# Edward-Sun/DIFUSCO

Hardware: NVIDIA H100
Metric: TSP-500 graphs/sec, 50-step categorical denoise (higher is better)
Workload: dtype f32 (3-term bf16 split on wgmma, fp32 accumulate)

## Files before the change

difusco_b200/csrc/edge_layer_tc.cuh:

```cuda
#pragma once
#include <cuda.h>
#include <cuda_bf16.h>
#include <cuda_runtime.h>

#include <stdlib.h>

#include <string>

#include "common.cuh"
#include "edge_layer_fp32.cuh"

namespace dfb {

constexpr int WG_ROWS = 64;
constexpr int TC_KCH = 64;
constexpr int TC_B_BYTES = 256 * 128;
constexpr int TC_A_CHUNK = WG_ROWS * 128;
constexpr int TC_A_BYTES = 8 * TC_A_CHUNK;
constexpr int CONV_BATCH = 16;

constexpr int W_LO_ROWS = H;
constexpr int W_MAT_ROWS = 2 * W_LO_ROWS;
constexpr int W_LAYER_ROWS = 6 * W_MAT_ROWS;
__host__ __device__ constexpr int w_row_C(int l) { return l * W_LAYER_ROWS; }
__host__ __device__ constexpr int w_row_O(int l) { return w_row_C(l) + W_MAT_ROWS; }
__host__ __device__ constexpr int w_row_UVAB(int l) { return w_row_C(l) + 2 * W_MAT_ROWS; }
__host__ __device__ constexpr int w_row_embed(int L, int which) { return L * W_LAYER_ROWS + which * W_MAT_ROWS; }
__host__ __device__ constexpr int w_arena_rows(int L) { return w_row_embed(L, 2); }

template <int NWG>
struct TcCfg {
  static_assert(NWG == 1 || NWG == 2, "one or two consumer warpgroups");
  static constexpr int TILE = NWG * WG_ROWS;
  static constexpr int THREADS = (NWG + 1) * 128;
  static constexpr int NSTAGE = (NWG == 1) ? 3 : 2;
  static constexpr int OFF_B = NWG * TC_A_BYTES;
  static constexpr int OFF_PRM = OFF_B + NSTAGE * TC_B_BYTES;
  static constexpr int OFF_ROW = OFF_PRM + 6 * H * 4;
  static constexpr int OFF_SRC = OFF_ROW + TILE * 4;
  static constexpr int OFF_BAR = OFF_SRC + TILE * 8;
  static constexpr int SMEM_BYTES = OFF_BAR + 2 * NSTAGE * 8;
  static constexpr int SMEM_ALLOC = SMEM_BYTES + 1024;
  static constexpr int OFF_TAU = SMEM_BYTES;
  static constexpr int SMEM_ALLOC_TROWS = SMEM_ALLOC + TILE * 8;
  static_assert(SMEM_ALLOC_TROWS <= 232448, "shared memory budget (227 KB per block)");
};

struct TcParams {
  float* e;
  const float* uvab;
  float* partials;
  GraphDev g;
  LayerParams lp;
  const float* tvec;
  const float* xt_lut;
  const float* lut;
  const float* zero_row;
  float* debug_acc;
  const float* lin_in;
  float* lin_out;
  const float* lin_bias;
  int lin_rows;
  int lin_nb;
  int lin_w_row;
  int* error_flag;
  unsigned long long* phase_cycles;
  int write_e, e_zero, agg_mode;
  int w_row_base;
  int n_tiles;
  TimeRows trows;
};

__device__ __forceinline__ uint32_t smem_u32(const void* p) { return (uint32_t)__cvta_generic_to_shared(p); }

__device__ __forceinline__ void mbar_init(uint64_t* bar, uint32_t count) {
  asm volatile("mbarrier.init.shared::cta.b64 [%0], %1;" ::"r"(smem_u32(bar)), "r"(count) : "memory");
}
__device__ __forceinline__ void mbar_arrive(uint64_t* bar) {
  asm volatile("mbarrier.arrive.shared::cta.b64 _, [%0];" ::"r"(smem_u32(bar)) : "memory");
}
__device__ __forceinline__ void mbar_arrive_expect_tx(uint64_t* bar, uint32_t bytes) {
  asm volatile("mbarrier.arrive.expect_tx.shared::cta.b64 _, [%0], %1;" ::"r"(smem_u32(bar)), "r"(bytes) : "memory");
}
__device__ __forceinline__ void mbar_wait(uint64_t* bar, uint32_t parity, int* error_flag, int code) {
  const uint32_t addr = smem_u32(bar);
  uint32_t ok = 0;
#pragma unroll 1
  for (uint32_t spin = 0;; ++spin) {
    asm volatile(
        "{\n .reg .pred p;\n mbarrier.try_wait.parity.shared::cta.b64 p, [%1], %2, %3;\n selp.u32 %0, 1, 0, p;\n}"
        : "=r"(ok)
        : "r"(addr), "r"(parity), "r"(20000u)
        : "memory");
    if (ok) return;
    if (spin > 400000u) {
      if (error_flag) {
        error_flag[1] = (int)blockIdx.x;
        error_flag[2] = (int)parity;
        error_flag[3] = (int)threadIdx.x;
        atomicExch(error_flag, code);
      }
      __threadfence_system();
      __trap();
    }
  }
}
__device__ __forceinline__ void tma_load_2d(uint32_t dst, const CUtensorMap* map, uint64_t* bar, int c0, int c1) {
  asm volatile(
      "cp.async.bulk.tensor.2d.shared::cluster.global.mbarrier::complete_tx::bytes [%0], [%1, {%3, %4}], [%2];"
      ::"r"(dst), "l"(reinterpret_cast<uint64_t>(map)), "r"(smem_u32(bar)), "r"(c0), "r"(c1)
      : "memory");
}
__device__ __forceinline__ void fence_proxy_async() { asm volatile("fence.proxy.async.shared::cta;" ::: "memory"); }
__device__ __forceinline__ void cp_async16(void* dst, const void* src) {
  asm volatile("cp.async.cg.shared.global [%0], [%1], 16;" ::"r"(smem_u32(dst)), "l"(src) : "memory");
}
__device__ __forceinline__ void cp_async_commit() { asm volatile("cp.async.commit_group;" ::: "memory"); }
__device__ __forceinline__ void cp_async_wait_all() { asm volatile("cp.async.wait_group 0;" ::: "memory"); }

__device__ __forceinline__ uint64_t wgmma_desc_sw128(uint32_t smem_addr) {
  return (uint64_t)((smem_addr >> 4) & 0x3fffu) | (1ull << 16) | (64ull << 32) | (1ull << 62);
}
__device__ __forceinline__ void wgmma_fence() { asm volatile("wgmma.fence.sync.aligned;" ::: "memory"); }
__device__ __forceinline__ void wgmma_commit() { asm volatile("wgmma.commit_group.sync.aligned;" ::: "memory"); }
template <int N>
__device__ __forceinline__ void wgmma_wait() { asm volatile("wgmma.wait_group.sync.aligned %0;" ::"n"(N) : "memory"); }
__device__ __forceinline__ void acc_fence(float (&d)[128]) {
#pragma unroll
  for (int i = 0; i < 128; ++i) asm volatile("" : "+f"(d[i])::"memory");
}
__device__ __forceinline__ void wgmma_bf16(float (&d)[128], uint64_t da, uint64_t db, uint32_t scale_d) {
  asm volatile(
      "{\n .reg .pred p;\n setp.ne.b32 p, %130, 0;\n"
      "wgmma.mma_async.sync.aligned.m64n256k16.f32.bf16.bf16 "
      "{%0, %1, %2, %3, %4, %5, %6, %7, %8, %9, %10, %11, %12, %13, %14, %15, "
      "%16, %17, %18, %19, %20, %21, %22, %23, %24, %25, %26, %27, %28, %29, %30, %31, "
      "%32, %33, %34, %35, %36, %37, %38, %39, %40, %41, %42, %43, %44, %45, %46, %47, "
      "%48, %49, %50, %51, %52, %53, %54, %55, %56, %57, %58, %59, %60, %61, %62, %63, "
      "%64, %65, %66, %67, %68, %69, %70, %71, %72, %73, %74, %75, %76, %77, %78, %79, "
      "%80, %81, %82, %83, %84, %85, %86, %87, %88, %89, %90, %91, %92, %93, %94, %95, "
      "%96, %97, %98, %99, %100, %101, %102, %103, %104, %105, %106, %107, %108, %109, %110, %111, "
      "%112, %113, %114, %115, %116, %117, %118, %119, %120, %121, %122, %123, %124, %125, %126, %127}, "
      "%128, %129, p, 1, 1, 0, 0;\n}"
      : "+f"(d[0]), "+f"(d[1]), "+f"(d[2]), "+f"(d[3]), "+f"(d[4]), "+f"(d[5]), "+f"(d[6]), "+f"(d[7]),
        "+f"(d[8]), "+f"(d[9]), "+f"(d[10]), "+f"(d[11]), "+f"(d[12]), "+f"(d[13]), "+f"(d[14]), "+f"(d[15]),
        "+f"(d[16]), "+f"(d[17]), "+f"(d[18]), "+f"(d[19]), "+f"(d[20]), "+f"(d[21]), "+f"(d[22]), "+f"(d[23]),
        "+f"(d[24]), "+f"(d[25]), "+f"(d[26]), "+f"(d[27]), "+f"(d[28]), "+f"(d[29]), "+f"(d[30]), "+f"(d[31]),
        "+f"(d[32]), "+f"(d[33]), "+f"(d[34]), "+f"(d[35]), "+f"(d[36]), "+f"(d[37]), "+f"(d[38]), "+f"(d[39]),
        "+f"(d[40]), "+f"(d[41]), "+f"(d[42]), "+f"(d[43]), "+f"(d[44]), "+f"(d[45]), "+f"(d[46]), "+f"(d[47]),
        "+f"(d[48]), "+f"(d[49]), "+f"(d[50]), "+f"(d[51]), "+f"(d[52]), "+f"(d[53]), "+f"(d[54]), "+f"(d[55]),
        "+f"(d[56]), "+f"(d[57]), "+f"(d[58]), "+f"(d[59]), "+f"(d[60]), "+f"(d[61]), "+f"(d[62]), "+f"(d[63]),
        "+f"(d[64]), "+f"(d[65]), "+f"(d[66]), "+f"(d[67]), "+f"(d[68]), "+f"(d[69]), "+f"(d[70]), "+f"(d[71]),
        "+f"(d[72]), "+f"(d[73]), "+f"(d[74]), "+f"(d[75]), "+f"(d[76]), "+f"(d[77]), "+f"(d[78]), "+f"(d[79]),
        "+f"(d[80]), "+f"(d[81]), "+f"(d[82]), "+f"(d[83]), "+f"(d[84]), "+f"(d[85]), "+f"(d[86]), "+f"(d[87]),
        "+f"(d[88]), "+f"(d[89]), "+f"(d[90]), "+f"(d[91]), "+f"(d[92]), "+f"(d[93]), "+f"(d[94]), "+f"(d[95]),
        "+f"(d[96]), "+f"(d[97]), "+f"(d[98]), "+f"(d[99]), "+f"(d[100]), "+f"(d[101]), "+f"(d[102]), "+f"(d[103]),
        "+f"(d[104]), "+f"(d[105]), "+f"(d[106]), "+f"(d[107]), "+f"(d[108]), "+f"(d[109]), "+f"(d[110]), "+f"(d[111]),
        "+f"(d[112]), "+f"(d[113]), "+f"(d[114]), "+f"(d[115]), "+f"(d[116]), "+f"(d[117]), "+f"(d[118]), "+f"(d[119]),
        "+f"(d[120]), "+f"(d[121]), "+f"(d[122]), "+f"(d[123]), "+f"(d[124]), "+f"(d[125]), "+f"(d[126]), "+f"(d[127])
      : "l"(da), "l"(db), "r"(scale_d));
}

__device__ __forceinline__ float sigmoid_mufu(float x) {
  float t, r;
  asm("ex2.approx.ftz.f32 %0, %1;" : "=f"(t) : "f"(-1.4426950408889634f * x));
  asm("rcp.approx.ftz.f32 %0, %1;" : "=f"(r) : "f"(1.0f + t));
  return r;
}
__device__ __forceinline__ void split4(float4 x, uint2& hi, uint2& lo) {
  __nv_bfloat162 h01 = __floats2bfloat162_rn(x.x, x.y), h23 = __floats2bfloat162_rn(x.z, x.w);
  float2 f01 = __bfloat1622float2(h01), f23 = __bfloat1622float2(h23);
  __nv_bfloat162 l01 = __floats2bfloat162_rn(x.x - f01.x, x.y - f01.y);
  __nv_bfloat162 l23 = __floats2bfloat162_rn(x.z - f23.x, x.w - f23.y);
  hi.x = *reinterpret_cast<uint32_t*>(&h01);
  hi.y = *reinterpret_cast<uint32_t*>(&h23);
  lo.x = *reinterpret_cast<uint32_t*>(&l01);
  lo.y = *reinterpret_cast<uint32_t*>(&l23);
}
__device__ __forceinline__ void split2(float a, float b, uint32_t& hi, uint32_t& lo) {
  __nv_bfloat162 h = __floats2bfloat162_rn(a, b);
  const float2 f = __bfloat1622float2(h);
  __nv_bfloat162 l = __floats2bfloat162_rn(a - f.x, b - f.y);
  hi = *reinterpret_cast<uint32_t*>(&h);
  lo = *reinterpret_cast<uint32_t*>(&l);
}
__device__ __forceinline__ uint32_t sw128_off(int r, int j) {
  return (uint32_t)((r >> 3) * 1024 + (r & 7) * 128 + ((j ^ (r & 7)) << 4));
}
__device__ __forceinline__ int msg_col(int j, int r) { return 64 * (j >> 3) + ((8 * (j & 7)) ^ (8 * (r & 7))); }
__device__ __forceinline__ float quad_sum(float v) {
  v += __shfl_xor_sync(0xffffffffu, v, 1);
  return v + __shfl_xor_sync(0xffffffffu, v, 2);
}
__device__ __forceinline__ void swap_row_halves(float (&d)[128]) {
#pragma unroll
  for (int j = 0; j < 32; ++j) {
    const float x0 = d[4 * j], x1 = d[4 * j + 1];
    d[4 * j] = d[4 * j + 2];
    d[4 * j + 1] = d[4 * j + 3];
    d[4 * j + 2] = x0;
    d[4 * j + 3] = x1;
  }
}

enum {
  PH_TILES = 0,
  PH_TOTAL,
  PH_CONVERT,
  PH_G1_WAIT,
  PH_G1_MMA,
  PH_E1,
  PH_REDUCE,
  PH_LN,
  PH_G2_WAIT,
  PH_G2_MMA,
  PH_E4,
  PH_COUNT
};

template <int NWG, bool LIN, bool TIMED = false, bool TROWS = false>
__device__ __forceinline__ void edge_layer_wg_body(const CUtensorMap& wmap, const TcParams& P) {
  using Cfg = TcCfg<NWG>;
  constexpr int NSTAGE = Cfg::NSTAGE;
  extern __shared__ unsigned char smem_raw[];
  unsigned char* smem = smem_raw + ((1024u - (smem_u32(smem_raw) & 1023u)) & 1023u);
  float* prm = reinterpret_cast<float*>(smem + Cfg::OFF_PRM);
  int* s_row = reinterpret_cast<int*>(smem + Cfg::OFF_ROW);
  const float** s_src = reinterpret_cast<const float**>(smem + Cfg::OFF_SRC);
  const float** s_tau = reinterpret_cast<const float**>(smem + Cfg::OFF_TAU);
  uint64_t* full = reinterpret_cast<uint64_t*>(smem + Cfg::OFF_BAR);
  uint64_t* empty = full + NSTAGE;

  const int warp = threadIdx.x >> 5, lane = threadIdx.x & 31;
  constexpr bool lin = LIN;
  const int loads_per_tile = (P.write_e ? 16 : 8) * NWG;

  if (threadIdx.x == 0) {
    for (int s = 0; s < NSTAGE; ++s) {
      mbar_init(&full[s], 1);
      mbar_init(&empty[s], 4);
    }
    asm volatile("fence.mbarrier_init.release.cluster;" ::: "memory");
    fence_proxy_async();
  }
  for (int i = threadIdx.x; i < H; i += Cfg::THREADS) {
    prm[i] = P.lp.ln_e_g[i];
    prm[H + i] = P.lp.ln_e_b[i];
    prm[2 * H + i] = P.tvec ? P.tvec[i] : 0.0f;
    prm[3 * H + i] = P.lp.ln_o_g[i];
    prm[4 * H + i] = P.lp.ln_o_b[i];
    prm[5 * H + i] = P.lp.b_O[i];
  }
  __syncthreads();
  const uint32_t smem_base = smem_u32(smem);

  if (warp >= 4 * NWG) {
    if constexpr (NWG == 2) asm volatile("setmaxnreg.dec.sync.aligned.u32 40;" ::: "memory");
    if (warp == 4 * NWG && lane == 0) {
      uint32_t u = 0;
      for (int tile = blockIdx.x; tile < P.n_tiles; tile += gridDim.x) {
        for (int i = 0; i < loads_per_tile; ++i, ++u) {
          const int s = u % NSTAGE;
          mbar_wait(&empty[s], ((u / NSTAGE) & 1) ^ 1, P.error_flag, 1);
          mbar_arrive_expect_tx(&full[s], TC_B_BYTES);
          const int row = (lin ? P.lin_w_row + (P.lin_nb == 4 ? (tile & 3) : 0) * W_MAT_ROWS
                               : P.w_row_base + (i >= 8 * NWG ? w_row_O(0) - w_row_C(0) : 0)) +
                          (i & 1) * W_LO_ROWS;
          tma_load_2d(smem_base + Cfg::OFF_B + s * TC_B_BYTES, &wmap, &full[s], ((i >> 1) & 3) * TC_KCH, row);
        }
      }
    }
    return;
  }

  if constexpr (NWG == 2) asm volatile("setmaxnreg.inc.sync.aligned.u32 232;" ::: "memory");
  const int wg = warp >> 2, wi = warp & 3, tid = threadIdx.x & 127;
  const int t4 = lane & 3;
  const int lr0 = wi * 16 + (lane >> 2);
  unsigned char* a_reg = smem + wg * TC_A_BYTES;
  const uint32_t a_base = smem_base + wg * TC_A_BYTES;
  float* msg = reinterpret_cast<float*>(a_reg);
  int* w_row = s_row + wg * WG_ROWS;
  const float** w_src = s_src + wg * WG_ROWS;
  const float** w_tau = s_tau + wg * WG_ROWS;
  auto wg_bar = [&] { asm volatile("bar.sync %0, 128;" ::"r"(1 + wg) : "memory"); };
  const int n_rows = lin ? P.lin_rows : P.g.E;
  uint32_t u = 0;
  float acc[128];

  auto turn_wait = [&] {
    if constexpr (NWG == 2) asm volatile("bar.sync %0, 256;" ::"r"(3 + wg) : "memory");
  };
  auto turn_pass = [&] {
    if constexpr (NWG == 2) asm volatile("bar.arrive %0, 256;" ::"r"(4 - wg) : "memory");
  };
  if (wg == 1) turn_pass();

  uint32_t t_mark = 0, t_start = 0;
  if constexpr (TIMED) t_start = t_mark = (uint32_t)clock();
  auto record = [&](int slot, uint32_t v) {
    if constexpr (TIMED) {
      if (tid == 0) atomicAdd(P.phase_cycles + slot, (unsigned long long)v);
    }
  };
  auto mark = [&](int slot) {
    if constexpr (TIMED) {
      const uint32_t now = (uint32_t)clock();
      record(slot, now - t_mark);
      t_mark = now;
    }
  };

  auto gemm = [&](int wait_slot, int mma_slot) {
    uint32_t waited = 0;
    turn_wait();
    if constexpr (TIMED) t_mark = (uint32_t)clock();
    acc_fence(acc);
    wgmma_fence();
    int s_prev = 0;
#pragma unroll
    for (int i = 0; i < 8; ++i, ++u) {
      const int s = u % NSTAGE;
      uint32_t w0 = 0;
      if constexpr (TIMED) w0 = (uint32_t)clock();
      mbar_wait(&full[s], (u / NSTAGE) & 1, P.error_flag, 2);
      if constexpr (TIMED) waited += (uint32_t)clock() - w0;
      const uint32_t b = smem_base + Cfg::OFF_B + s * TC_B_BYTES;
      const uint32_t ahi = a_base + (i >> 1) * 2 * TC_A_CHUNK, alo = ahi + TC_A_CHUNK;
#pragma unroll
      for (int ks = 0; ks < 4; ++ks) {
        const uint64_t db = wgmma_desc_sw128(b + ks * 32);
        wgmma_bf16(acc, wgmma_desc_sw128(ahi + ks * 32), db, (i | ks) ? 1u : 0u);
        if ((i & 1) == 0) wgmma_bf16(acc, wgmma_desc_sw128(alo + ks * 32), db, 1u);
      }
      wgmma_commit();
      if (i > 0) {
        wgmma_wait<1>();
        __syncwarp();
        if (lane == 0) mbar_arrive(&empty[s_prev]);
      }
      s_prev = s;
    }
    wgmma_wait<0>();
    acc_fence(acc);
    __syncwarp();
    if (lane == 0) mbar_arrive(&empty[s_prev]);
    turn_pass();
    if constexpr (TIMED) {
      const uint32_t now = (uint32_t)clock();
      record(wait_slot, waited);
      record(mma_slot, now - t_mark - waited);
      t_mark = now;
    }
  };

  auto stage_rows = [&](auto row_src) {
#pragma unroll 1
    for (int i = 0; i < 16; ++i) {
      const int r = wi * 16 + i;
      const float* src = row_src(i) + 4 * lane;
      float* dst = msg + r * H + ((4 * lane) ^ (8 * (r & 7)));
      cp_async16(dst, src);
      cp_async16(dst + 128, src + 128);
    }
    cp_async_commit();
  };

  for (int tile = blockIdx.x; tile < P.n_tiles; tile += gridDim.x) {
    record(PH_TILES, 1);
    const int row_tile = (lin && P.lin_nb == 4) ? (tile >> 2) : tile;
    const int s_base = row_tile * Cfg::TILE + wg * WG_ROWS;
    if (tid < WG_ROWS) {
      const int s = s_base + tid;
      const float* src = P.zero_row;
      int rw = -1;
      if (s < n_rows && lin) {
        src = P.lin_in + (size_t)s * H;
      } else if (s < n_rows) {
        rw = P.g.row[s];
        if (P.e_zero) src = P.zero_row;
        else if (P.xt_lut) src = P.lut + ((P.xt_lut[P.g.perm ? P.g.perm[s] : s] != 0.0f) ? H : 0);
        else src = P.e + (size_t)s * H;
      }
      w_row[tid] = rw;
      w_src[tid] = src;
      if constexpr (TROWS) w_tau[tid] = s < n_rows ? time_row(P.tvec, P.trows, P.g.perm ? P.g.perm[s] : s) : P.zero_row;
    }
    wg_bar();

#pragma unroll 1
    for (int it0 = 0; it0 < 32; it0 += CONV_BATCH) {
      float4 x[CONV_BATCH];
#pragma unroll
      for (int q = 0; q < CONV_BATCH; ++q) {
        const int item = (it0 + q) * 128 + tid;
        x[q] = __ldcg(reinterpret_cast<const float4*>(w_src[item >> 6]) + (item & 63));
      }
#pragma unroll
      for (int q = 0; q < CONV_BATCH; ++q) {
        const int item = (it0 + q) * 128 + tid;
        const int rr = item >> 6, k4 = item & 63;
        uint2 hi, lo;
        split4(x[q], hi, lo);
        const uint32_t off = (k4 >> 4) * 2 * TC_A_CHUNK + sw128_off(rr, (k4 & 15) >> 1) + (k4 & 1) * 8;
        *reinterpret_cast<uint2*>(a_reg + off) = hi;
        *reinterpret_cast<uint2*>(a_reg + off + TC_A_CHUNK) = lo;
      }
    }
    fence_proxy_async();
    wg_bar();
    mark(PH_CONVERT);
    gemm(PH_G1_WAIT, PH_G1_MMA);

    const int sa = s_base + lr0, sb = sa + 8;
    const bool va = sa < n_rows, vb = sb < n_rows;
    if (lin || P.debug_acc) {
      const int nb = (lin && P.lin_nb == 4) ? (tile & 3) : 0;
      const int ostride = lin ? P.lin_nb * H : H;
      float* out = lin ? P.lin_out + nb * H : P.debug_acc;
#pragma unroll
      for (int h = 0; h < 2; ++h) {
        const int s = h ? sb : sa;
        if (!(h ? vb : va)) continue;
#pragma unroll
        for (int j = 0; j < 32; ++j) {
          const int c = 8 * j + 2 * t4;
          float2 o = make_float2(acc[4 * j + 2 * h], acc[4 * j + 2 * h + 1]);
          if (lin) {
            const float2 bb = __ldg(reinterpret_cast<const float2*>(P.lin_bias + nb * H + c));
            o.x += bb.x;
            o.y += bb.y;
          }
          __stcg(reinterpret_cast<float2*>(out + (size_t)s * ostride + c), o);
        }
      }
      continue;
    }

    const int s_lane = s_base + wi * 16 + (lane & 15);
    const int col_lane = s_lane < n_rows ? P.g.col[s_lane] : 0;
    stage_rows([&](int i) { return P.uvab + (size_t)__shfl_sync(0xffffffffu, col_lane, i) * 4 * H + H; });
#pragma unroll 1
    for (int h = 0; h < 2; ++h) {
      const bool v = h ? vb : va;
      const float* ap = P.uvab + (size_t)__shfl_sync(0xffffffffu, col_lane, (lane >> 2) + 8 * h) * 4 * H + 2 * H;
      const float* bp = P.uvab + (size_t)(v ? P.g.row[h ? sb : sa] : 0) * 4 * H + 3 * H;
#pragma unroll
      for (int j = 0; j < 32; ++j) {
        const int c = 8 * j + 2 * t4;
        const float2 ah = __ldg(reinterpret_cast<const float2*>(ap + c));
        const float2 bh = __ldg(reinterpret_cast<const float2*>(bp + c));
        acc[4 * j] = (acc[4 * j] + ah.x) + bh.x;
        acc[4 * j + 1] = (acc[4 * j + 1] + ah.y) + bh.y;
      }
      if (h == 0) {
        cp_async_wait_all();
        __syncwarp();
      }
      float* m = msg + (lr0 + 8 * h) * H + 2 * t4;
#pragma unroll
      for (int j = 0; j < 32; ++j) {
        float2* mp = reinterpret_cast<float2*>(m + msg_col(j, lr0));
        const float2 vh = *mp;
        *mp = make_float2(sigmoid_mufu(acc[4 * j]) * vh.x, sigmoid_mufu(acc[4 * j + 1]) * vh.y);
      }
      swap_row_halves(acc);
    }
    wg_bar();
    mark(PH_E1);
    const bool amax = P.agg_mode == AGG_MAX;
    const float run0 = amax ? -INFINITY : 0.0f;
#pragma unroll 1
    for (int g2 = 0; g2 < WG_ROWS / GROUP; ++g2) {
      const int grp = (s_base >> 5) + g2;
      if (grp >= P.g.n_groups) break;
      const int first_node = P.g.grp_first[grp];
      const size_t pair_base = (size_t)P.g.grp_pair[grp];
      const int node = w_row[g2 * GROUP + lane];
      const int nxt = __shfl_down_sync(0xffffffffu, node, 1);
      const uint32_t ends = __ballot_sync(0xffffffffu, node >= 0 && (lane == GROUP - 1 || nxt != node));
#pragma unroll 1
      for (int cc = 0; cc < 2; ++cc) {
        const int c = tid + 128 * cc;
        float run = run0;
#pragma unroll 8
        for (int r = 0; r < GROUP; ++r) {
          const int lr = g2 * GROUP + r;
          const float m = msg[lr * H + (c ^ (8 * (lr & 7)))];
          run = amax ? fmaxf(run, m) : run + m;
          if ((ends >> r) & 1u) {
            P.partials[(pair_base + (size_t)(w_row[lr] - first_node)) * H + c] = run;
            run = run0;
          }
        }
      }
    }
    wg_bar();
    mark(PH_REDUCE);
    if (!P.write_e) continue;

#pragma unroll 1
    for (int h = 0; h < 2; ++h) {
      float sum = 0.f;
#pragma unroll
      for (int j = 0; j < 32; ++j) sum += acc[4 * j] + acc[4 * j + 1];
      float mean = quad_sum(sum) * (1.0f / H);
      float q = 0.f;
#pragma unroll
      for (int j = 0; j < 32; ++j) {
        const float d0 = acc[4 * j] - mean, d1 = acc[4 * j + 1] - mean;
        q = fmaf(d0, d0, fmaf(d1, d1, q));
      }
      float rstd = rsqrtf(quad_sum(q) * (1.0f / H) + LN_EPS);
      sum = 0.f;
      const float* tau = nullptr;
      if constexpr (TROWS) tau = w_tau[lr0 + 8 * h];
#pragma unroll
      for (int j = 0; j < 32; ++j) {
        const int c = 8 * j + 2 * t4;
        const float2 g = *reinterpret_cast<const float2*>(prm + c);
        const float2 b = *reinterpret_cast<const float2*>(prm + H + c);
        float2 t;
        if constexpr (TROWS) t = __ldg(reinterpret_cast<const float2*>(tau + c));
        else t = *reinterpret_cast<const float2*>(prm + 2 * H + c);
        const float y0 = fmaxf(fmaf((acc[4 * j] - mean) * rstd, g.x, b.x), 0.0f) + t.x;
        const float y1 = fmaxf(fmaf((acc[4 * j + 1] - mean) * rstd, g.y, b.y), 0.0f) + t.y;
        acc[4 * j] = y0;
        acc[4 * j + 1] = y1;
        sum += y0 + y1;
      }
      mean = quad_sum(sum) * (1.0f / H);
      q = 0.f;
#pragma unroll
      for (int j = 0; j < 32; ++j) {
        const float d0 = acc[4 * j] - mean, d1 = acc[4 * j + 1] - mean;
        q = fmaf(d0, d0, fmaf(d1, d1, q));
      }
      rstd = rsqrtf(quad_sum(q) * (1.0f / H) + LN_EPS);
      const int r = lr0 + 8 * h;
#pragma unroll
      for (int j = 0; j < 32; ++j) {
        const int c = 8 * j + 2 * t4;
        const float2 g = *reinterpret_cast<const float2*>(prm + 3 * H + c);
        const float2 b = *reinterpret_cast<const float2*>(prm + 4 * H + c);
        const float z0 = fmaf((acc[4 * j] - mean) * rstd, g.x, b.x);
        const float z1 = fmaf((acc[4 * j + 1] - mean) * rstd, g.y, b.y);
        uint32_t hi, lo;
        split2(z0 * sigmoid_mufu(z0), z1 * sigmoid_mufu(z1), hi, lo);
        const uint32_t off = (j >> 3) * 2 * TC_A_CHUNK + sw128_off(r, j & 7) + 4 * t4;
        *reinterpret_cast<uint32_t*>(a_reg + off) = hi;
        *reinterpret_cast<uint32_t*>(a_reg + off + TC_A_CHUNK) = lo;
      }
      swap_row_halves(acc);
    }
    const float* e_src = w_src[wi * 16 + (lane & 15)];
    fence_proxy_async();
    wg_bar();
    mark(PH_LN);
    gemm(PH_G2_WAIT, PH_G2_MMA);

    stage_rows([&](int i) {
      return reinterpret_cast<const float*>(__shfl_sync(0xffffffffu, reinterpret_cast<unsigned long long>(e_src), i));
    });
    cp_async_wait_all();
    __syncwarp();
#pragma unroll
    for (int h = 0; h < 2; ++h) {
      if (!(h ? vb : va)) continue;
      const int r = lr0 + 8 * h;
      const float* er = msg + r * H + 2 * t4;
      float* dst = P.e + (size_t)(h ? sb : sa) * H;
#pragma unroll
      for (int j = 0; j < 32; ++j) {
        const int c = 8 * j + 2 * t4;
        const float2 ein = *reinterpret_cast<const float2*>(er + msg_col(j, r));
        const float2 bo = *reinterpret_cast<const float2*>(prm + 5 * H + c);
        __stcg(reinterpret_cast<float2*>(dst + c),
               make_float2((ein.x + acc[4 * j + 2 * h]) + bo.x, (ein.y + acc[4 * j + 2 * h + 1]) + bo.y));
      }
    }
    mark(PH_E4);
  }
  if constexpr (TIMED) record(PH_TOTAL, (uint32_t)clock() - t_start);
}

__global__ void __launch_bounds__(TcCfg<2>::THREADS, 1)
k_edge_layer_wg2(const __grid_constant__ CUtensorMap wmap, const TcParams P) {
  edge_layer_wg_body<2, false>(wmap, P);
}
__global__ void __launch_bounds__(TcCfg<2>::THREADS, 1)
k_edge_layer_wg2_timed(const __grid_constant__ CUtensorMap wmap, const TcParams P) {
  edge_layer_wg_body<2, false, true>(wmap, P);
}
__global__ void __launch_bounds__(TcCfg<1>::THREADS, 1)
k_edge_layer_wg1(const __grid_constant__ CUtensorMap wmap, const TcParams P) {
  edge_layer_wg_body<1, false>(wmap, P);
}
__global__ void __launch_bounds__(TcCfg<2>::THREADS, 1)
k_edge_layer_wg2_trows(const __grid_constant__ CUtensorMap wmap, const TcParams P) {
  edge_layer_wg_body<2, false, false, true>(wmap, P);
}
__global__ void __launch_bounds__(TcCfg<1>::THREADS, 1)
k_edge_layer_wg1_trows(const __grid_constant__ CUtensorMap wmap, const TcParams P) {
  edge_layer_wg_body<1, false, false, true>(wmap, P);
}
__global__ void __launch_bounds__(TcCfg<2>::THREADS, 1)
k_linear_wg2(const __grid_constant__ CUtensorMap wmap, const TcParams P) {
  edge_layer_wg_body<2, true>(wmap, P);
}

struct TcState {
  std::string err;
  int num_sms = 0;
  CUtensorMap wmap;
  bool bound = false;
  float* zero_row = nullptr;
  int* error_flag = nullptr;
  int* error_host = nullptr;
  unsigned long long* phase_cycles = nullptr;

  TcState() = default;
  TcState(const TcState&) = delete;
  TcState& operator=(const TcState&) = delete;
  ~TcState() {
    if (zero_row) cudaFree(zero_row);
    if (error_host) cudaFreeHost(error_host);
    if (phase_cycles) cudaFree(phase_cycles);
  }
};

typedef CUresult (*PFN_encodeTiled)(CUtensorMap*, CUtensorMapDataType, cuuint32_t, void*, const cuuint64_t*,
                                    const cuuint64_t*, const cuuint32_t*, const cuuint32_t*, CUtensorMapInterleave,
                                    CUtensorMapSwizzle, CUtensorMapL2promotion, CUtensorMapFloatOOBfill);

inline int tc_init(TcState* st, int num_sms) {
  st->num_sms = num_sms;
  cudaError_t e = cudaFuncSetAttribute(k_edge_layer_wg2, cudaFuncAttributeMaxDynamicSharedMemorySize, TcCfg<2>::SMEM_ALLOC);
  if (e == cudaSuccess)
    e = cudaFuncSetAttribute(k_edge_layer_wg2_timed, cudaFuncAttributeMaxDynamicSharedMemorySize, TcCfg<2>::SMEM_ALLOC);
  if (e == cudaSuccess)
    e = cudaFuncSetAttribute(k_edge_layer_wg1, cudaFuncAttributeMaxDynamicSharedMemorySize, TcCfg<1>::SMEM_ALLOC);
  if (e == cudaSuccess)
    e = cudaFuncSetAttribute(k_edge_layer_wg2_trows, cudaFuncAttributeMaxDynamicSharedMemorySize, TcCfg<2>::SMEM_ALLOC_TROWS);
  if (e == cudaSuccess)
    e = cudaFuncSetAttribute(k_edge_layer_wg1_trows, cudaFuncAttributeMaxDynamicSharedMemorySize, TcCfg<1>::SMEM_ALLOC_TROWS);
  if (e == cudaSuccess)
    e = cudaFuncSetAttribute(k_linear_wg2, cudaFuncAttributeMaxDynamicSharedMemorySize, TcCfg<2>::SMEM_ALLOC);
  if (e != cudaSuccess) {
    st->err = std::string("cudaFuncSetAttribute: ") + cudaGetErrorString(e);
    return -2;
  }
  if ((e = cudaMalloc(&st->zero_row, H * sizeof(float))) != cudaSuccess ||
      (e = cudaMemset(st->zero_row, 0, H * sizeof(float))) != cudaSuccess ||
      (e = cudaMalloc(&st->phase_cycles, 32 * sizeof(unsigned long long))) != cudaSuccess ||
      (e = cudaMemset(st->phase_cycles, 0, 32 * sizeof(unsigned long long))) != cudaSuccess ||
      (e = cudaHostAlloc(&st->error_host, 4 * sizeof(int), cudaHostAllocMapped)) != cudaSuccess ||
      (e = cudaHostGetDevicePointer((void**)&st->error_flag, st->error_host, 0)) != cudaSuccess) {
    st->err = std::string("tc_init alloc: ") + cudaGetErrorString(e);
    return -2;
  }
  return 0;
}

inline int tc_bind_weights(TcState* st, const uint16_t* arena, int L) {
  void* fn = nullptr;
  cudaDriverEntryPointQueryResult qres;
  cudaError_t e = cudaGetDriverEntryPoint("cuTensorMapEncodeTiled", &fn, cudaEnableDefault, &qres);
  if (e != cudaSuccess || !fn || qres != cudaDriverEntryPointSuccess) {
    st->err = "cuTensorMapEncodeTiled entry point not available";
    cudaGetLastError();
    return -2;
  }
  cuuint64_t gdim[2] = {(cuuint64_t)H, (cuuint64_t)w_arena_rows(L)};
  cuuint64_t gstride[1] = {(cuuint64_t)H * sizeof(uint16_t)};
  cuuint32_t box[2] = {(cuuint32_t)TC_KCH, 256u};
  cuuint32_t estr[2] = {1u, 1u};
  CUresult r = ((PFN_encodeTiled)fn)(&st->wmap, CU_TENSOR_MAP_DATA_TYPE_BFLOAT16, 2, (void*)arena, gdim,
                                     gstride, box, estr, CU_TENSOR_MAP_INTERLEAVE_NONE, CU_TENSOR_MAP_SWIZZLE_128B,
                                     CU_TENSOR_MAP_L2_PROMOTION_L2_256B, CU_TENSOR_MAP_FLOAT_OOB_FILL_NONE);
  if (r != CUDA_SUCCESS) {
    st->err = "cuTensorMapEncodeTiled failed with CUresult " + std::to_string((int)r);
    return -2;
  }
  st->bound = true;
  return 0;
}

template <int NWG>
inline int tc_launch(TcState* st, void (*kernel)(CUtensorMap, TcParams), TcParams& P, int rows, int nb,
                     cudaStream_t stream, int smem = TcCfg<NWG>::SMEM_ALLOC) {
  if (!st->bound) {
    st->err = "weights not bound";
    return -1;
  }
  P.zero_row = st->zero_row; P.error_flag = st->error_flag; P.phase_cycles = st->phase_cycles;
  P.n_tiles = nb * ((rows + TcCfg<NWG>::TILE - 1) / TcCfg<NWG>::TILE);
  const int grid = P.n_tiles < st->num_sms ? P.n_tiles : st->num_sms;
  kernel<<<grid, TcCfg<NWG>::THREADS, smem, stream>>>(st->wmap, P);
  const cudaError_t err = cudaGetLastError();
  if (err == cudaSuccess) return 0;
  st->err = std::string("launch: ") + cudaGetErrorString(err);
  return -2;
}

inline int tc_launch_edge_layer(TcState* st, int l, float* e, const float* uvab, float* partials, const GraphDev& g,
                                const LayerParams& lp, const float* tvec, const TimeRows& trows, int write_e,
                                int e_zero, const float* xt_lut, const float* lut, int agg_mode, int nwg, bool timed,
                                float* debug_acc, cudaStream_t stream) {
  TcParams P{};
  P.e = e; P.uvab = uvab; P.partials = partials; P.g = g; P.lp = lp; P.tvec = tvec;
  P.xt_lut = xt_lut; P.lut = lut; P.debug_acc = debug_acc;
  P.write_e = debug_acc ? 0 : write_e;
  P.e_zero = e_zero; P.agg_mode = agg_mode;
  P.w_row_base = w_row_C(l);
  if (trows.index && tvec && !debug_acc) {
    P.trows = trows;
    if (nwg == 1) return tc_launch<1>(st, k_edge_layer_wg1_trows, P, g.E, 1, stream, TcCfg<1>::SMEM_ALLOC_TROWS);
    return tc_launch<2>(st, k_edge_layer_wg2_trows, P, g.E, 1, stream, TcCfg<2>::SMEM_ALLOC_TROWS);
  }
  if (nwg == 1) return tc_launch<1>(st, k_edge_layer_wg1, P, g.E, 1, stream);
  return tc_launch<2>(st, timed && !debug_acc ? k_edge_layer_wg2_timed : k_edge_layer_wg2, P, g.E, 1, stream);
}

inline int tc_launch_linear(TcState* st, const float* in, float* out, const float* bias, int rows, int nb, int w_row,
                            cudaStream_t stream) {
  TcParams P{};
  P.lin_in = in; P.lin_out = out; P.lin_bias = bias; P.lin_rows = rows; P.lin_nb = nb; P.lin_w_row = w_row;
  P.lp.ln_e_g = P.lp.ln_e_b = P.lp.ln_o_g = P.lp.ln_o_b = P.lp.b_O = st->zero_row;
  return tc_launch<2>(st, k_linear_wg2, P, rows, nb, stream);
}

}
```

Before: 22.44.

## Split weight TMA chunks into 32-wide K slices with a four-stage ring

```diff
diff --git a/difusco_b200/csrc/edge_layer_tc.cuh b/difusco_b200/csrc/edge_layer_tc.cuh
--- a/difusco_b200/csrc/edge_layer_tc.cuh
+++ b/difusco_b200/csrc/edge_layer_tc.cuh
@@ -13,8 +13,10 @@
 namespace dfb {
 
 constexpr int WG_ROWS = 64;
-constexpr int TC_KCH = 64;
-constexpr int TC_B_BYTES = 256 * 128;
+constexpr int TC_KBLK = 64;
+constexpr int TC_KCH = 32;
+constexpr int TC_B_BYTES = 256 * TC_KCH * 2;
+static_assert(TC_KCH * 2 == 64, "weight chunk rows are one 64-byte swizzle row (tensor map, wgmma_desc_sw64)");
 constexpr int TC_A_CHUNK = WG_ROWS * 128;
 constexpr int TC_A_BYTES = 8 * TC_A_CHUNK;
 constexpr int CONV_BATCH = 16;
@@ -33,7 +35,7 @@
   static_assert(NWG == 1 || NWG == 2, "one or two consumer warpgroups");
   static constexpr int TILE = NWG * WG_ROWS;
   static constexpr int THREADS = (NWG + 1) * 128;
-  static constexpr int NSTAGE = (NWG == 1) ? 3 : 2;
+  static constexpr int NSTAGE = 2 * TC_KBLK / TC_KCH;
   static constexpr int OFF_B = NWG * TC_A_BYTES;
   static constexpr int OFF_PRM = OFF_B + NSTAGE * TC_B_BYTES;
   static constexpr int OFF_ROW = OFF_PRM + 6 * H * 4;
@@ -120,6 +122,9 @@
 
 __device__ __forceinline__ uint64_t wgmma_desc_sw128(uint32_t smem_addr) {
   return (uint64_t)((smem_addr >> 4) & 0x3fffu) | (1ull << 16) | (64ull << 32) | (1ull << 62);
+}
+__device__ __forceinline__ uint64_t wgmma_desc_sw64(uint32_t smem_addr) {
+  return (uint64_t)((smem_addr >> 4) & 0x3fffu) | (1ull << 16) | (32ull << 32) | (2ull << 62);
 }
 __device__ __forceinline__ void wgmma_fence() { asm volatile("wgmma.fence.sync.aligned;" ::: "memory"); }
 __device__ __forceinline__ void wgmma_commit() { asm volatile("wgmma.commit_group.sync.aligned;" ::: "memory"); }
@@ -233,7 +238,7 @@
 
   const int warp = threadIdx.x >> 5, lane = threadIdx.x & 31;
   constexpr bool lin = LIN;
-  const int loads_per_tile = (P.write_e ? 16 : 8) * NWG;
+  const int loads_per_tile = (P.write_e ? 2 : 1) * NWG * 4 * NSTAGE;
 
   if (threadIdx.x == 0) {
     for (int s = 0; s < NSTAGE; ++s) {
@@ -264,9 +269,10 @@
           mbar_wait(&empty[s], ((u / NSTAGE) & 1) ^ 1, P.error_flag, 1);
           mbar_arrive_expect_tx(&full[s], TC_B_BYTES);
           const int row = (lin ? P.lin_w_row + (P.lin_nb == 4 ? (tile & 3) : 0) * W_MAT_ROWS
-                               : P.w_row_base + (i >= 8 * NWG ? w_row_O(0) - w_row_C(0) : 0)) +
-                          (i & 1) * W_LO_ROWS;
-          tma_load_2d(smem_base + Cfg::OFF_B + s * TC_B_BYTES, &wmap, &full[s], ((i >> 1) & 3) * TC_KCH, row);
+                               : P.w_row_base + (i >= 4 * NSTAGE * NWG ? w_row_O(0) - w_row_C(0) : 0)) +
+                          (s >= NSTAGE / 2 ? W_LO_ROWS : 0);
+          const int k = ((i / NSTAGE) & 3) * TC_KBLK + (s % (NSTAGE / 2)) * TC_KCH;
+          tma_load_2d(smem_base + Cfg::OFF_B + s * TC_B_BYTES, &wmap, &full[s], k, row);
         }
       }
     }
@@ -285,7 +291,6 @@
   const float** w_tau = s_tau + wg * WG_ROWS;
   auto wg_bar = [&] { asm volatile("bar.sync %0, 128;" ::"r"(1 + wg) : "memory"); };
   const int n_rows = lin ? P.lin_rows : P.g.E;
-  uint32_t u = 0;
   float acc[128];
 
   auto turn_wait = [&] {
@@ -317,34 +322,34 @@
     if constexpr (TIMED) t_mark = (uint32_t)clock();
     acc_fence(acc);
     wgmma_fence();
-    int s_prev = 0;
-#pragma unroll
-    for (int i = 0; i < 8; ++i, ++u) {
-      const int s = u % NSTAGE;
-      uint32_t w0 = 0;
-      if constexpr (TIMED) w0 = (uint32_t)clock();
-      mbar_wait(&full[s], (u / NSTAGE) & 1, P.error_flag, 2);
-      if constexpr (TIMED) waited += (uint32_t)clock() - w0;
-      const uint32_t b = smem_base + Cfg::OFF_B + s * TC_B_BYTES;
-      const uint32_t ahi = a_base + (i >> 1) * 2 * TC_A_CHUNK, alo = ahi + TC_A_CHUNK;
-#pragma unroll
-      for (int ks = 0; ks < 4; ++ks) {
-        const uint64_t db = wgmma_desc_sw128(b + ks * 32);
-        wgmma_bf16(acc, wgmma_desc_sw128(ahi + ks * 32), db, (i | ks) ? 1u : 0u);
-        if ((i & 1) == 0) wgmma_bf16(acc, wgmma_desc_sw128(alo + ks * 32), db, 1u);
-      }
-      wgmma_commit();
-      if (i > 0) {
+#pragma unroll 1
+    for (int kc = 0; kc < 4; ++kc) {
+      const uint32_t ahi = a_base + kc * 2 * TC_A_CHUNK, alo = ahi + TC_A_CHUNK;
+#pragma unroll
+      for (int s = 0; s < NSTAGE; ++s) {
+        uint32_t w0 = 0;
+        if constexpr (TIMED) w0 = (uint32_t)clock();
+        mbar_wait(&full[s], kc & 1, P.error_flag, 2);
+        if constexpr (TIMED) waited += (uint32_t)clock() - w0;
+        const uint32_t b = smem_base + Cfg::OFF_B + s * TC_B_BYTES;
+        const bool b_hi = s < NSTAGE / 2;
+#pragma unroll
+        for (int k = 0; k < TC_KCH / 16; ++k) {
+          const int ks = (s % (NSTAGE / 2)) * (TC_KCH / 16) + k;
+          const uint64_t db = wgmma_desc_sw64(b + k * 32);
+          wgmma_bf16(acc, wgmma_desc_sw128(ahi + ks * 32), db, (b_hi && ks == 0) ? (uint32_t)(kc != 0) : 1u);
+          if (b_hi) wgmma_bf16(acc, wgmma_desc_sw128(alo + ks * 32), db, 1u);
+        }
+        wgmma_commit();
         wgmma_wait<1>();
         __syncwarp();
-        if (lane == 0) mbar_arrive(&empty[s_prev]);
-      }
-      s_prev = s;
+        if (lane == 0 && (s > 0 || kc > 0)) mbar_arrive(&empty[(s + NSTAGE - 1) % NSTAGE]);
+      }
     }
     wgmma_wait<0>();
     acc_fence(acc);
     __syncwarp();
-    if (lane == 0) mbar_arrive(&empty[s_prev]);
+    if (lane == 0) mbar_arrive(&empty[NSTAGE - 1]);
     turn_pass();
     if constexpr (TIMED) {
       const uint32_t now = (uint32_t)clock();
@@ -676,7 +681,7 @@
   cuuint32_t box[2] = {(cuuint32_t)TC_KCH, 256u};
   cuuint32_t estr[2] = {1u, 1u};
   CUresult r = ((PFN_encodeTiled)fn)(&st->wmap, CU_TENSOR_MAP_DATA_TYPE_BFLOAT16, 2, (void*)arena, gdim,
-                                     gstride, box, estr, CU_TENSOR_MAP_INTERLEAVE_NONE, CU_TENSOR_MAP_SWIZZLE_128B,
+                                     gstride, box, estr, CU_TENSOR_MAP_INTERLEAVE_NONE, CU_TENSOR_MAP_SWIZZLE_64B,
                                      CU_TENSOR_MAP_L2_PROMOTION_L2_256B, CU_TENSOR_MAP_FLOAT_OOB_FILL_NONE);
   if (r != CUDA_SUCCESS) {
     st->err = "cuTensorMapEncodeTiled failed with CUresult " + std::to_string((int)r);
```

After: 23.45, median of 6. 1.05x the previous value.
